# insight-platform/Similari

Hardware: NVIDIA H100
Metric: pair_associations_per_sec (higher is better)
Workload: dtype f32

## Files before the change

### similari_b200/csrc/kernels_feat_tc.cu

```cuda
#include <cuda.h>
#include <cuda_bf16.h>
#include <cuda_runtime.h>
#include <stdint.h>

#include <algorithm>
#include <cstdlib>
#include <cstring>

#include "sb_engine.cuh"
#include "sb_tc.cuh"

namespace sb {

constexpr int TC_STAGES = 4;
constexpr int TC_STAGE_BYTES = TC_A_BYTES + TC_B_BYTES;

struct TcHdr { int scene, m0, ncols_left, m, det_base, col0, epoch, vis_lbase, vis_lcap, pad; };
struct TcSmem {
  unsigned char stage[TC_STAGES][TC_STAGE_BYTES];
  VisColMeta meta[4][TC_BN];
  VisRowMeta rowm[4][TC_BM];
  float colb[4][TC_BN];
  unsigned int colvalid[4][TC_BN / 32];
  TcHdr hdr[4];
  unsigned long long full_bar[TC_STAGES];
  unsigned long long empty_bar[TC_STAGES];
  unsigned long long meta_full[4];
  unsigned long long meta_empty[4];
};
static_assert(sizeof(TcSmem) + 1024 <= 227 * 1024, "screen kernel exceeds the shared memory of an SM");


template <bool COSINE>
__global__ void __launch_bounds__(TC_THREADS, 1)
vis_screen_kernel(const __grid_constant__ CUtensorMap mapA, const __grid_constant__ CUtensorMap mapB, Params p,
                  TrackStore ts, Frame f, const TcTile* tiles, int n_tiles_host, const int* n_tiles_dev,
                  const VisColMeta* colmeta, const VisColGeo* colgeo, const VisRowMeta* rowmeta, const float* colb,
                  const unsigned int* colvalid) {
  const int n_tiles = n_tiles_dev ? *n_tiles_dev : n_tiles_host;
  extern __shared__ unsigned char smem_raw_[];
  TcSmem& S = *reinterpret_cast<TcSmem*>(smem_raw_ + ((1024u - (smem_u32(smem_raw_) & 1023u)) & 1023u));
  const int warp = threadIdx.x >> 5, lane = threadIdx.x & 31;
  const int K = p.max_obs;
  const int KB = (p.d8 + TC_BK - 1) / TC_BK;

  unsigned char* const stage_base = &S.stage[0][0];
  const uint32_t crank = cluster_rank();
  const int cta_first = (int)(blockIdx.x >> 1);
  const int cta_step = (int)(gridDim.x >> 1);
  if (threadIdx.x == 0) {
    for (int s = 0; s < TC_STAGES; ++s) { mbar_init(&S.full_bar[s], 1); mbar_init(&S.empty_bar[s], 4); }
    for (int b = 0; b < 4; ++b) { mbar_init(&S.meta_full[b], 1); mbar_init(&S.meta_empty[b], 8); }
    asm volatile("fence.mbarrier_init.release.cluster;" ::: "memory");
  }
  __syncthreads();
  cluster_sync_all();

  if (warp < 4) {
    asm volatile("setmaxnreg.dec.sync.aligned.u32 40;");
    if (warp == 0 && lane == 0) {
      asm volatile("prefetch.tensormap [%0];" ::"l"((uint64_t)&mapA) : "memory");
      asm volatile("prefetch.tensormap [%0];" ::"l"((uint64_t)&mapB) : "memory");
      int stage = 0;
      uint32_t phase = 0;
      int it = 0;
      TcTile tl_n;
      tl_n.scene = 0; tl_n.m0 = 0; tl_n.c0 = 0; tl_n.pad = 0;
      if (cta_first < n_tiles) tl_n = tiles[cta_first];
      SceneDesc sc_n = f.scenes[tl_n.scene];
      for (int t = cta_first; t < n_tiles; t += cta_step, ++it) {
        const TcTile tl = tl_n;
        const SceneDesc sc = sc_n;
        if (t + cta_step < n_tiles) { tl_n = tiles[t + cta_step]; sc_n = f.scenes[tl_n.scene]; }
        const int m0 = tl.m0 + (int)crank * TC_BM;
        const int rowA = sc.det_base + m0;
        const int rowB = sc.slot * ts.track_cap * K + tl.c0;
        {
          const int g = it & 3;
          mbar_wait(&S.meta_empty[g], ((it >> 2) & 1) ^ 1);
          TcHdr h;
          h.scene = tl.scene; h.m0 = m0; h.ncols_left = sc.nb * K - tl.c0; h.m = sc.m; h.det_base = sc.det_base;
          h.col0 = sc.col_off + tl.c0; h.epoch = (int)sc.epoch; h.vis_lbase = sc.vis_lbase; h.vis_lcap = sc.vis_lcap; h.pad = 0;
          S.hdr[g] = h;
          mbar_expect_tx(&S.meta_full[g], (uint32_t)(sizeof(VisColMeta) * TC_BN + sizeof(VisRowMeta) * TC_BM +
                                                    4 * TC_BN + TC_BN / 8));
          bulk_load(S.meta[g], colmeta + h.col0, (uint32_t)(sizeof(VisColMeta) * TC_BN), &S.meta_full[g]);
          bulk_load(S.rowm[g], rowmeta + rowA, (uint32_t)(sizeof(VisRowMeta) * TC_BM), &S.meta_full[g]);
          bulk_load(S.colb[g], colb + h.col0, 4 * TC_BN, &S.meta_full[g]);
          bulk_load(S.colvalid[g], colvalid + (h.col0 >> 5), TC_BN / 8, &S.meta_full[g]);
        }
        for (int kb = 0; kb < KB; ++kb) {
          mbar_wait(&S.empty_bar[stage], phase ^ 1);
          unsigned char* base = stage_base + stage * TC_STAGE_BYTES;
          mbar_expect_tx(&S.full_bar[stage], TC_STAGE_BYTES);
          tma_load_2d(base, &mapA, kb * TC_BK, rowA, &S.full_bar[stage]);
          tma_load_2d_mc(base + TC_A_BYTES + crank * (TC_B_BYTES / 2), &mapB, kb * TC_BK, rowB + (int)crank * (TC_BN / 2),
                         &S.full_bar[stage], (uint16_t)0x3);
          if (++stage == TC_STAGES) { stage = 0; phase ^= 1; }
        }
      }
    }
  } else {
    asm volatile("setmaxnreg.inc.sync.aligned.u32 232;");
    const int wg = (warp >> 2) - 1;
    const int rr[2] = {wg * TC_WG_ROWS + (warp & 3) * 16 + (lane >> 2), wg * TC_WG_ROWS + (warp & 3) * 16 + (lane >> 2) + 8};
    const int q2 = 2 * (lane & 3);
    const bool geo = p.n_constraints > 0;
    int stage = 0;
    uint32_t phase = 0;
    int it = 0;
    for (int t = cta_first; t < n_tiles; t += cta_step, ++it) {
      float acc[128];
      tc_consume_tile<2, TC_STAGES, TC_STAGE_BYTES>(acc, stage_base, S.full_bar, S.empty_bar, KB, wg, stage, phase);
      const int ms = it & 3;
      mbar_wait(&S.meta_full[ms], (it >> 2) & 1);
      const VisColMeta* gmeta = S.meta[ms];
      const TcHdr h = S.hdr[ms];
      const float* gcolb = S.colb[ms];
      float rowk[2];
      bool row_ok[2];
      int g[2];
#pragma unroll
      for (int hr = 0; hr < 2; ++hr) {
        const VisRowMeta rm = S.rowm[ms][rr[hr]];
        const int m = h.m0 + rr[hr];
        row_ok[hr] = m < h.m && rm.ok;
        g[hr] = h.det_base + m;
        rowk[hr] = rm.rowk;
      }
      unsigned int keep[4] = {0u, 0u, 0u, 0u};
#pragma unroll
      for (int j = 0; j < TC_BN / 8; ++j) {
        const int c0 = 8 * j + q2;
        const float2 cb = *reinterpret_cast<const float2*>(gcolb + c0);
        const unsigned int vw = S.colvalid[ms][c0 >> 5] >> (c0 & 31);
#pragma unroll
        for (int e = 0; e < 4; ++e) {
          const int hr = e >> 1, cl = e & 1;
          const float b = COSINE ? rowk[hr] * (cl ? cb.y : cb.x) : rowk[hr] + (cl ? cb.y : cb.x);
          const bool k = !(acc[4 * j + e] < b) && ((vw >> cl) & 1u) && c0 + cl < h.ncols_left && row_ok[hr];
          if (k) keep[j >> 3] |= 1u << (((4 * j) & 31) + e);
        }
      }
      if (geo) {
        float cx[2], cy[2], cr[2];
#pragma unroll
        for (int hr = 0; hr < 2; ++hr) {
          cx[hr] = 0.0f; cy[hr] = 0.0f; cr[hr] = 0.0f;
          if (row_ok[hr]) { cx[hr] = f.c_box[(size_t)g[hr] * 6]; cy[hr] = f.c_box[(size_t)g[hr] * 6 + 1]; cr[hr] = f.c_radius[g[hr]]; }
        }
#pragma unroll
        for (int w = 0; w < 4; ++w) {
          unsigned int kk = keep[w];
          while (kk) {
            const int b = __ffs(kk) - 1;
            kk &= kk - 1;
            const int i = w * 32 + b, hr = (i >> 1) & 1;
            const int col = 8 * (i >> 2) + q2 + (i & 1);
            const VisColGeo cg = colgeo[h.col0 + col];
            if (!compat_ok(p, (unsigned int)h.epoch, cg.tep, cx[hr], cy[hr], cr[hr], cg.tx, cg.ty, cg.tr)) keep[w] &= ~(1u << b);
          }
        }
      }
      int cnt = 0;
#pragma unroll
      for (int w = 0; w < 4; ++w) cnt += __popc(keep[w]);
      if (__any_sync(0xffffffffu, cnt != 0)) {
        int incl = cnt;
#pragma unroll
        for (int o = 1; o < 32; o <<= 1) {
          int tt = __shfl_up_sync(0xffffffffu, incl, o);
          if (lane >= o) incl += tt;
        }
        const int total = __shfl_sync(0xffffffffu, incl, 31);
        int base = 0;
        if (lane == 31) base = atomicAdd(&f.vis_cnt[h.scene], total);
        base = __shfl_sync(0xffffffffu, base, 31);
        int pos = base + incl - cnt;
#pragma unroll
        for (int hr = 0; hr < 2; ++hr) {
#pragma unroll
          for (int w = 0; w < 4; ++w) {
            unsigned int kk = keep[w] & (hr ? 0xccccccccu : 0x33333333u);
            while (kk) {
              const int b = __ffs(kk) - 1;
              kk &= kk - 1;
              if (pos < h.vis_lcap) {
                const int i = w * 32 + b;
                const VisColMeta cm = gmeta[8 * (i >> 2) + q2 + (i & 1)];
                VisPair vp;
                vp.g = g[hr]; vp.row = cm.row; vp.scene = h.scene; vp.outcol = cm.outcol;
                f.vis_pairs[h.vis_lbase + pos] = vp;
              }
              ++pos;
            }
          }
        }
      }
      __syncwarp();
      if (lane == 0) mbar_arrive(&S.meta_empty[ms]);
    }
  }
  __syncthreads();
  cluster_sync_all();
}

constexpr int SA_BN = 128;
constexpr int SA_KMAX = 8;
constexpr int SA_A_BLOCK = TC_BM * TC_BK * 2;
constexpr int SA_B_STAGE = SA_BN * TC_BK * 2;
constexpr int SA_STAGES = 5;
constexpr int SA_SLABS = 4;
struct SaHdr { int scene, m0, ncols, m, det_base, col0, epoch, vis_lbase, vis_lcap, unit, last, pad; };
struct SaSmem {
  unsigned char a[SA_KMAX][SA_A_BLOCK];
  unsigned char b[SA_STAGES][SA_B_STAGE];
  VisColMeta meta[SA_SLABS][SA_BN];
  float colb[SA_SLABS][SA_BN];
  float colsb[SA_SLABS][SA_BN];
  unsigned int colvalid[SA_SLABS][SA_BN / 32];
  SaHdr hdr[SA_SLABS];
  unsigned long long a_full[SA_KMAX];
  unsigned long long a_empty;
  unsigned long long full_bar[SA_STAGES];
  unsigned long long empty_bar[SA_STAGES];
  unsigned long long meta_full[SA_SLABS];
  unsigned long long meta_empty[SA_SLABS];
};
static_assert(sizeof(SaSmem) + 1024 <= 227 * 1024, "A-stationary screen kernel exceeds the shared memory of an SM");
constexpr int kScreenStationaryMaxD8 = SA_KMAX * TC_BK;

template <bool COSINE, bool FP8>
__global__ void __launch_bounds__(TC_THREADS, 1)
vis_screen_sa_kernel(const __grid_constant__ CUtensorMap mapA, const __grid_constant__ CUtensorMap mapB, Params p,
                     TrackStore ts, Frame f, const TcTile* units, int n_units_host, const int* n_units_dev, int ucols,
                     const VisColMeta* colmeta, const VisColGeo* colgeo, const VisRowMeta* rowmeta, const float* colb,
                     const float* colsb, const unsigned int* colvalid) {
  constexpr bool kScaled = FP8 && !COSINE;
  constexpr int BKF = FP8 ? 2 * TC_BK : TC_BK;
  const int n_units = n_units_dev ? *n_units_dev : n_units_host;
  extern __shared__ unsigned char smem_raw_[];
  SaSmem& S = *reinterpret_cast<SaSmem*>(smem_raw_ + ((1024u - (smem_u32(smem_raw_) & 1023u)) & 1023u));
  const int warp = threadIdx.x >> 5, lane = threadIdx.x & 31;
  const int K = p.max_obs;
  const int KB = (p.d8 + BKF - 1) / BKF;
  const uint32_t crank = cluster_rank();
  if (threadIdx.x == 0) {
    for (int kb = 0; kb < SA_KMAX; ++kb) mbar_init(&S.a_full[kb], 1);
    mbar_init(&S.a_empty, 2);
    for (int s = 0; s < SA_STAGES; ++s) { mbar_init(&S.full_bar[s], 1); mbar_init(&S.empty_bar[s], 2); }
    for (int b = 0; b < SA_SLABS; ++b) { mbar_init(&S.meta_full[b], 1); mbar_init(&S.meta_empty[b], 4); }
    asm volatile("fence.mbarrier_init.release.cluster;" ::: "memory");
  }
  __syncthreads();
  cluster_sync_all();

  if (warp < 4) {
    asm volatile("setmaxnreg.dec.sync.aligned.u32 40;");
    if (warp == 0 && lane == 0) {
      asm volatile("prefetch.tensormap [%0];" ::"l"((uint64_t)&mapA) : "memory");
      asm volatile("prefetch.tensormap [%0];" ::"l"((uint64_t)&mapB) : "memory");
      int seq = 0, gk = 0, unit = 0;
      for (int u = (int)(blockIdx.x >> 1); u < n_units; u += (int)(gridDim.x >> 1), ++unit) {
        const TcTile tl = units[u];
        const SceneDesc sc = f.scenes[tl.scene];
        const int m0 = tl.m0 + (int)crank * TC_BM;
        const int rowA = sc.det_base + m0;
        const int cols = min(ucols, sc.nb * K - tl.c0);
        const int nct = (cols + SA_BN - 1) / SA_BN;
        const int rowB = sc.slot * ts.track_cap * K + tl.c0;
        if (unit > 0) mbar_wait(&S.a_empty, (unit - 1) & 1);
        if (nct == 1) mbar_arrive(&S.a_empty);
        for (int ct = 0; ct < nct; ++ct, ++seq) {
          const int g = seq % SA_SLABS;
          mbar_wait(&S.meta_empty[g], ((seq / SA_SLABS) & 1) ^ 1);
          SaHdr h;
          h.scene = tl.scene; h.m0 = m0; h.ncols = min(SA_BN, cols - ct * SA_BN); h.m = sc.m; h.det_base = sc.det_base;
          h.col0 = sc.col_off + tl.c0 + ct * SA_BN; h.epoch = (int)sc.epoch; h.vis_lbase = sc.vis_lbase;
          h.vis_lcap = sc.vis_lcap; h.unit = unit; h.last = ct + 2 >= nct; h.pad = 0;
          S.hdr[g] = h;
          mbar_expect_tx(&S.meta_full[g], (uint32_t)(sizeof(VisColMeta) * SA_BN + (kScaled ? 8 : 4) * SA_BN + SA_BN / 8));
          bulk_load(S.meta[g], colmeta + h.col0, (uint32_t)(sizeof(VisColMeta) * SA_BN), &S.meta_full[g]);
          bulk_load(S.colb[g], colb + h.col0, 4 * SA_BN, &S.meta_full[g]);
          if (kScaled) bulk_load(S.colsb[g], colsb + h.col0, 4 * SA_BN, &S.meta_full[g]);
          bulk_load(S.colvalid[g], colvalid + (h.col0 >> 5), SA_BN / 8, &S.meta_full[g]);
          for (int kb = 0; kb < KB; ++kb, ++gk) {
            if (ct == 0) {
              mbar_expect_tx(&S.a_full[kb], SA_A_BLOCK);
              tma_load_2d(S.a[kb], &mapA, kb * BKF, rowA, &S.a_full[kb]);
            }
            const int s = gk % SA_STAGES;
            mbar_wait(&S.empty_bar[s], ((gk / SA_STAGES) & 1) ^ 1);
            mbar_expect_tx(&S.full_bar[s], SA_B_STAGE);
            tma_load_2d_mc(S.b[s] + crank * (SA_B_STAGE / 2), &mapB, kb * BKF, rowB + ct * SA_BN + (int)crank * (SA_BN / 2),
                           &S.full_bar[s], (uint16_t)0x3);
          }
        }
      }
      for (int e = 0; e < 2; ++e, ++seq) {
        const int g = seq % SA_SLABS;
        mbar_wait(&S.meta_empty[g], ((seq / SA_SLABS) & 1) ^ 1);
        S.hdr[g].scene = -1 - e;
        mbar_arrive(&S.meta_full[g]);
      }
    }
  } else {
    asm volatile("setmaxnreg.inc.sync.aligned.u32 232;");
    const int wg = (warp >> 2) - 1;
    const int rr[2] = {(warp & 3) * 16 + (lane >> 2), (warp & 3) * 16 + (lane >> 2) + 8};
    const int q2 = 2 * (lane & 3);
    const bool geo = p.n_constraints > 0;
    const bool elected = (threadIdx.x & 127) == 0;
    for (int pos = wg;; pos += 2) {
      const int ms = pos % SA_SLABS;
      mbar_wait(&S.meta_full[ms], (pos / SA_SLABS) & 1);
      const SaHdr h = S.hdr[ms];
      if (pos > 0) wg2_bar_sync(1 + (pos & 1));
      if (h.scene < 0) {
        if (h.scene == -1) wg2_bar_arrive(1 + ((pos + 1) & 1));
        break;
      }
      float rowk[2][2], rowi[2][2];
      bool row_ok[2][2];
#pragma unroll
      for (int hh = 0; hh < 2; ++hh)
#pragma unroll
        for (int hr = 0; hr < 2; ++hr) {
          const int m = h.m0 + 64 * hh + rr[hr];
          const VisRowMeta rm = rowmeta[h.det_base + m];
          rowk[hh][hr] = rm.rowk;
          rowi[hh][hr] = rm.rowi;
          row_ok[hh][hr] = m < h.m && rm.ok;
        }

      float acc[128];
      {
        const int g0 = pos * KB;
        int stage = g0 % SA_STAGES;
        uint32_t phase = (g0 / SA_STAGES) & 1;
        int prev = -1;
        auto release = [&](int s) {
          if (elected)
            for (uint32_t r = 0; r < 2; ++r) mbar_arrive_cluster(cluster_addr(&S.empty_bar[s], r));
        };
        for (int kb = 0; kb < KB; ++kb) {
          mbar_wait(&S.a_full[kb], (uint32_t)h.unit & 1u);
          mbar_wait(&S.full_bar[stage], phase);
          const uint32_t a0 = smem_u32(S.a[kb]);
          const uint32_t b0 = smem_u32(S.b[stage]);
          wgmma_fence();
#pragma unroll
          for (int k = 0; k < 4; ++k) {
            const uint32_t acc_on = (kb | k) != 0 ? 1u : 0u;
            if (FP8) {
              wgmma_e4m3_m64n128(acc, wgmma_desc(a0 + k * 32), wgmma_desc(b0 + k * 32), acc_on);
              wgmma_e4m3_m64n128(acc + 64, wgmma_desc(a0 + 64 * 128 + k * 32), wgmma_desc(b0 + k * 32), acc_on);
            } else {
              wgmma_bf16_m64n128(acc, wgmma_desc(a0 + k * 32), wgmma_desc(b0 + k * 32), acc_on);
              wgmma_bf16_m64n128(acc + 64, wgmma_desc(a0 + 64 * 128 + k * 32), wgmma_desc(b0 + k * 32), acc_on);
            }
          }
          wgmma_commit();
          wgmma_wait<1>();
          if (prev >= 0) release(prev);
          prev = stage;
          if (++stage == SA_STAGES) { stage = 0; phase ^= 1; }
        }
        wg2_bar_arrive(1 + ((pos + 1) & 1));
        wgmma_wait<0>();
        wgmma_fence_acc(acc);
        release(prev);
        if (h.last && elected) mbar_arrive(&S.a_empty);
      }

      const VisColMeta* gmeta = S.meta[ms];
      const float* gcolb = S.colb[ms];
      unsigned int colm[2] = {0u, 0u};
#pragma unroll
      for (int j = 0; j < SA_BN / 8; ++j) {
        const int c0 = 8 * j + q2;
        unsigned int m2 = (S.colvalid[ms][c0 >> 5] >> (c0 & 31)) & 3u;
        m2 &= (c0 < h.ncols ? 1u : 0u) | (c0 + 1 < h.ncols ? 2u : 0u);
        colm[j >> 3] |= (m2 | (m2 << 2)) << ((4 * j) & 31);
      }
      unsigned int keep[4];
#pragma unroll
      for (int hh = 0; hh < 2; ++hh) {
        const unsigned int rowm = (row_ok[hh][0] ? 0x33333333u : 0u) | (row_ok[hh][1] ? 0xccccccccu : 0u);
        keep[2 * hh] = 0u;
        keep[2 * hh + 1] = 0u;
#pragma unroll
        for (int j = 0; j < SA_BN / 8; ++j) {
          const float2 cb = *reinterpret_cast<const float2*>(gcolb + 8 * j + q2);
          float2 cs = make_float2(1.0f, 1.0f);
          if (kScaled) cs = *reinterpret_cast<const float2*>(&S.colsb[ms][8 * j + q2]);
#pragma unroll
          for (int e = 0; e < 4; ++e) {
            const float rk = rowk[hh][e >> 1], c = (e & 1) ? cb.y : cb.x;
            if (kScaled) {
              const float b = __fmaf_rn((e & 1) ? cs.y : cs.x, rk, c);
              if (!(acc[64 * hh + 4 * j + e] * rowi[hh][e >> 1] < b)) keep[2 * hh + (j >> 3)] |= 1u << ((4 * j + e) & 31);
            } else {
              const float b = COSINE ? rk * c : rk + c;
              if (!(acc[64 * hh + 4 * j + e] < b)) keep[2 * hh + (j >> 3)] |= 1u << ((4 * j + e) & 31);
            }
          }
        }
        keep[2 * hh] &= colm[0] & rowm;
        keep[2 * hh + 1] &= colm[1] & rowm;
      }
      if (geo) {
        float cx[2][2], cy[2][2], cr[2][2];
#pragma unroll
        for (int hh = 0; hh < 2; ++hh)
#pragma unroll
          for (int hr = 0; hr < 2; ++hr) {
            cx[hh][hr] = 0.0f; cy[hh][hr] = 0.0f; cr[hh][hr] = 0.0f;
            if (row_ok[hh][hr]) {
              const size_t g = (size_t)h.det_base + h.m0 + 64 * hh + rr[hr];
              cx[hh][hr] = f.c_box[g * 6]; cy[hh][hr] = f.c_box[g * 6 + 1]; cr[hh][hr] = f.c_radius[g];
            }
          }
#pragma unroll
        for (int w = 0; w < 4; ++w) {
          unsigned int kk = keep[w];
          while (kk) {
            const int b = __ffs(kk) - 1;
            kk &= kk - 1;
            const int i = (w & 1) * 32 + b, hh = w >> 1;
            const bool r8 = (i >> 1) & 1;
            const int col = 8 * (i >> 2) + q2 + (i & 1);
            const VisColGeo cg = colgeo[h.col0 + col];
            if (!compat_ok(p, (unsigned int)h.epoch, cg.tep, r8 ? cx[hh][1] : cx[hh][0], r8 ? cy[hh][1] : cy[hh][0],
                           r8 ? cr[hh][1] : cr[hh][0], cg.tx, cg.ty, cg.tr))
              keep[w] &= ~(1u << b);
          }
        }
      }
      int cnt = 0;
#pragma unroll
      for (int w = 0; w < 4; ++w) cnt += __popc(keep[w]);
      if (__any_sync(0xffffffffu, cnt != 0)) {
        int incl = cnt;
#pragma unroll
        for (int o = 1; o < 32; o <<= 1) {
          int tt = __shfl_up_sync(0xffffffffu, incl, o);
          if (lane >= o) incl += tt;
        }
        const int total = __shfl_sync(0xffffffffu, incl, 31);
        int base = 0;
        if (lane == 31) base = atomicAdd(&f.vis_cnt[h.scene], total);
        base = __shfl_sync(0xffffffffu, base, 31);
        int at = base + incl - cnt;
#pragma unroll
        for (int hh = 0; hh < 2; ++hh) {
#pragma unroll
          for (int hr = 0; hr < 2; ++hr) {
            const int g = h.det_base + h.m0 + 64 * hh + rr[hr];
#pragma unroll
            for (int w = 0; w < 2; ++w) {
              unsigned int kk = keep[2 * hh + w] & (hr ? 0xccccccccu : 0x33333333u);
              while (kk) {
                const int b = __ffs(kk) - 1;
                kk &= kk - 1;
                if (at < h.vis_lcap) {
                  const int i = w * 32 + b;
                  const VisColMeta cm = gmeta[8 * (i >> 2) + q2 + (i & 1)];
                  VisPair vp;
                  vp.g = g; vp.row = cm.row; vp.scene = h.scene; vp.outcol = cm.outcol;
                  f.vis_pairs[h.vis_lbase + at] = vp;
                }
                ++at;
              }
            }
          }
        }
      }
      __syncwarp();
      if (lane == 0) mbar_arrive(&S.meta_empty[ms]);
    }
  }
  __syncthreads();
  cluster_sync_all();
}


constexpr int RF_WARPS = 4;
constexpr int RF_SEG = 64;
constexpr int RF_PITCH = RF_SEG + 1;
constexpr int RF_CLAIM = 16;

template <bool TAIL>
__device__ __forceinline__ void refine_load_a(const float* __restrict__ a, int blk, int D, float* av) {
  if (!TAIL) {
    const float4 a0 = *reinterpret_cast<const float4*>(a + blk * 8);
    const float4 a1 = *reinterpret_cast<const float4*>(a + blk * 8 + 4);
    av[0] = a0.x; av[1] = a0.y; av[2] = a0.z; av[3] = a0.w; av[4] = a1.x; av[5] = a1.y; av[6] = a1.z; av[7] = a1.w;
  } else {
#pragma unroll
    for (int l = 0; l < 8; ++l) av[l] = blk * 8 + l < D ? a[blk * 8 + l] : 0.0f;
  }
}
template <bool TAIL, class T>
__device__ __forceinline__ void refine_load_a(const T* __restrict__ a, int blk, int D, float* av) {
  if (!TAIL) {
    feat_widen8(*reinterpret_cast<const uint4*>(a + blk * 8), a, av);
  } else {
#pragma unroll
    for (int l = 0; l < 8; ++l) av[l] = blk * 8 + l < D ? feat_elem(a, blk * 8 + l) : 0.0f;
  }
}
template <bool COSINE>
__device__ __forceinline__ float refine_block_sum(const float* av, const float* __restrict__ b, int blk) {
  const float4 b0 = *reinterpret_cast<const float4*>(b + blk * 8);
  const float4 b1 = *reinterpret_cast<const float4*>(b + blk * 8 + 4);
  const float bb[8] = {b0.x, b0.y, b0.z, b0.w, b1.x, b1.y, b1.z, b1.w};
  float t[8];
#pragma unroll
  for (int l = 0; l < 8; ++l) {
    if (COSINE) t[l] = av[l] * bb[l];
    else { const float df = av[l] - bb[l]; t[l] = df * df; }
  }
  return reduce_add8(t);
}

template <bool COSINE, bool TAIL, class T>
__global__ void __launch_bounds__(RF_WARPS * 32, 8) vis_refine_kernel(Params p, TrackStore ts, Frame f, int* nan_flag,
                                                                      int n_scenes) {
  __shared__ float s_bs[RF_WARPS][RF_CLAIM][RF_PITCH];
  __shared__ int s_cnt[2];
  for (int scene = blockIdx.y; scene < n_scenes; scene += gridDim.y) {
    if (f.vis_mode[scene] != 0) {
      if (f.screen_cnt && blockIdx.x == 0 && threadIdx.x == 0) atomicAdd(f.screen_cnt + 2, 1);
      continue;
    }
    const SceneDesc sc = f.scenes[scene];
    const int lane = threadIdx.x & 31, w = threadIdx.x >> 5;
    if (f.screen_cnt) {
      if (threadIdx.x < 2) s_cnt[threadIdx.x] = 0;
      __syncthreads();
    }
    int n_ref = 0, n_cut = 0;
    const int n_pairs = min(f.vis_cnt[scene], sc.vis_lcap);
    const int nblk = p.d8 / 8;
    const int D = p.feature_dim;
    float (*bs)[RF_PITCH] = s_bs[w];
    float vmax = nanf("");
    for (;;) {
      int i0 = 0;
      if (lane == 0) i0 = atomicAdd(f.refine_next + scene, RF_CLAIM);
      i0 = __shfl_sync(0xffffffffu, i0, 0);
      if (i0 >= n_pairs) break;
      const int npair = min(RF_CLAIM, n_pairs - i0);
      VisPair mine;
      mine.g = 0; mine.row = 0; mine.scene = 0; mine.outcol = 0;
      if (lane < npair) mine = f.vis_pairs[sc.vis_lbase + i0 + lane];
      float acc = 0.0f;
      for (int seg0 = 0; seg0 < nblk; seg0 += RF_SEG) {
        const int segn = min(RF_SEG, nblk - seg0);
        int g_prev = -1;
        float av[RF_SEG / 32][8];
#pragma unroll 4
        for (int pp = 0; pp < npair; ++pp) {
          const int g = __shfl_sync(0xffffffffu, mine.g, pp);
          const int row = __shfl_sync(0xffffffffu, mine.row, pp);
          const float* b = ts.feat + (size_t)row * p.d8;
          if (g != g_prev) {
            const T* a = static_cast<const T*>(f.in_feat) + (size_t)g * D;
#pragma unroll
            for (int h = 0; h < RF_SEG / 32; ++h)
              if (h * 32 + lane < segn) refine_load_a<TAIL>(a, seg0 + h * 32 + lane, D, av[h]);
            g_prev = g;
          }
#pragma unroll
          for (int h = 0; h < RF_SEG / 32; ++h) {
            const int j = h * 32 + lane;
            if (j < segn) bs[pp][j] = refine_block_sum<COSINE>(av[h], b, seg0 + j);
          }
        }
        __syncwarp();
        if (lane < npair)
          for (int j = 0; j < segn; ++j) acc = acc + bs[lane][j];
        __syncwarp();
      }
      if (lane < npair) {
        float v = nanf("");
        if (COSINE) {
          const float d = acc / sqrtf(f.c_norm2[mine.g] * ts.fnorm2[mine.row]);
          if (d >= p.visual_threshold) v = 1.0f - d;
        } else {
          const float d = sqrtf(acc);
          if (d <= p.visual_threshold) v = d;
        }
        f.vis_val[sc.vis_lbase + i0 + lane] = v;
        n_ref += 1;
        n_cut += is_nan(v) ? 1 : 0;
        if (!is_nan(v) && !(v <= vmax)) vmax = v;
        if (nan_flag && is_nan(v)) nan_flag[scene] = 1;
      }
    }
    unsigned int u = 0u;
    if (!is_nan(vmax)) {
      u = __float_as_uint(vmax);
      u = (u & 0x80000000u) ? ~u : (u | 0x80000000u);
    }
#pragma unroll
    for (int o = 16; o > 0; o >>= 1) u = max(u, __shfl_xor_sync(0xffffffffu, u, o));
    if (lane == 0 && u != 0u) atomicMax(f.scene_max + scene, u);
    if (f.screen_cnt) {
      n_ref = __reduce_add_sync(0xffffffffu, n_ref);
      n_cut = __reduce_add_sync(0xffffffffu, n_cut);
      if (lane == 0 && n_ref) { atomicAdd(&s_cnt[0], n_ref); atomicAdd(&s_cnt[1], n_cut); }
      __syncthreads();
      if (threadIdx.x == 0 && s_cnt[0]) { atomicAdd(f.screen_cnt, s_cnt[0]); if (s_cnt[1]) atomicAdd(f.screen_cnt + 1, s_cnt[1]); }
      __syncthreads();
    }
  }
}

__global__ void vis_fill_none_kernel(Params p, Frame f, int n_scenes) {
  for (int scene = blockIdx.y; scene < n_scenes; scene += gridDim.y) {
    if (f.scene_mode[scene] != 0) continue;
    const SceneDesc sc = f.scenes[scene];
    const long long cnt = (long long)sc.m * sc.n * p.max_obs;
    float* out = f.vis + sc.vis_off;
    const float qnan = nanf("");
    for (long long i = (long long)blockIdx.x * blockDim.x + threadIdx.x; i < cnt; i += (long long)gridDim.x * blockDim.x) out[i] = qnan;
  }
}
__global__ void vis_scatter_kernel(Params p, Frame f, int n_scenes) {
  for (int scene = blockIdx.y; scene < n_scenes; scene += gridDim.y) {
    if (f.scene_mode[scene] != 0) continue;
    const SceneDesc sc = f.scenes[scene];
    const int n_pairs = min(f.vis_cnt[scene], sc.vis_lcap);
    float* out = f.vis + sc.vis_off;
    for (int i = blockIdx.x * blockDim.x + threadIdx.x; i < n_pairs; i += gridDim.x * blockDim.x) {
      const VisPair vp = f.vis_pairs[sc.vis_lbase + i];
      out[(size_t)(vp.g - sc.det_base) * (sc.n * p.max_obs) + vp.outcol] = f.vis_val[sc.vis_lbase + i];
    }
  }
}
void launch_vis_densify(const Params& p, const Frame& f, int n_scenes, cudaStream_t st) {
  if (n_scenes == 0) return;
  dim3 grid(64, scene_grid(n_scenes));
  vis_fill_none_kernel<<<grid, 256, 0, st>>>(p, f, n_scenes);
  vis_scatter_kernel<<<grid, 256, 0, st>>>(p, f, n_scenes);
  note_launch(2);
}

__global__ void to_bf16_kernel(const float* src, int src_pitch, int d, int d8, long long rows, __nv_bfloat16* dst) {
  long long i = (long long)blockIdx.x * blockDim.x + threadIdx.x;
  if (i >= rows * d8) return;
  long long r = i / d8;
  int c = (int)(i - r * d8);
  float x = c < d ? src[r * src_pitch + c] : 0.0f;
  dst[i] = __float2bfloat16_rn(x);
}

void launch_to_bf16(const float* src, int src_pitch, int d, int d8, long long rows, void* dst, cudaStream_t st) {
  if (rows == 0) return;
  long long n = rows * d8;
  to_bf16_kernel<<<(unsigned)((n + 255) / 256), 256, 0, st>>>(src, src_pitch, d, d8, rows, (__nv_bfloat16*)dst);
  note_launch();
}

__global__ void to_fp8_kernel(const float* src, int src_pitch, int d, int d8, long long rows, unsigned char* dst, float* scale) {
  const long long r = ((long long)blockIdx.x * blockDim.x + threadIdx.x) >> 5;
  if (r >= rows) return;
  const float s = fp8_row_from(src + r * src_pitch, d, d8, dst + r * fp8_pitch(d8));
  if ((threadIdx.x & 31) == 0) scale[r] = s;
}

void launch_to_fp8(const float* src, int src_pitch, int d, int d8, long long rows, unsigned char* dst, float* scale,
                   cudaStream_t st) {
  if (rows == 0) return;
  to_fp8_kernel<<<(unsigned)((rows * 32 + 255) / 256), 256, 0, st>>>(src, src_pitch, d, d8, rows, dst, scale);
  note_launch();
}

typedef CUresult (*EncodeTiledFn)(CUtensorMap*, CUtensorMapDataType, cuuint32_t, void*, const cuuint64_t*, const cuuint64_t*,
                                  const cuuint32_t*, const cuuint32_t*, CUtensorMapInterleave, CUtensorMapSwizzle,
                                  CUtensorMapL2promotion, CUtensorMapFloatOOBfill);

static EncodeTiledFn get_encode() {
  static EncodeTiledFn fn = nullptr;
  if (!fn) {
    void* p = nullptr;
    cudaDriverEntryPointQueryResult qr;
    if (cudaGetDriverEntryPoint("cuTensorMapEncodeTiled", &p, cudaEnableDefault, &qr) == cudaSuccess && p) fn = (EncodeTiledFn)p;
  }
  return fn;
}

int make_map(CUtensorMap* m, const void* base, long long rows, int d8, int box_rows, bool fp8) {
  EncodeTiledFn enc = get_encode();
  if (!enc) return -1;
  cuuint64_t dims[2] = {(cuuint64_t)d8, (cuuint64_t)rows};
  cuuint64_t strides[1] = {fp8 ? (cuuint64_t)fp8_pitch(d8) : (cuuint64_t)d8 * 2};
  cuuint32_t box[2] = {(cuuint32_t)(fp8 ? 2 * TC_BK : TC_BK), (cuuint32_t)box_rows};
  cuuint32_t estr[2] = {1, 1};
  CUresult r = enc(m, fp8 ? CU_TENSOR_MAP_DATA_TYPE_UINT8 : CU_TENSOR_MAP_DATA_TYPE_BFLOAT16, 2, (void*)base, dims, strides, box, estr, CU_TENSOR_MAP_INTERLEAVE_NONE,
                   CU_TENSOR_MAP_SWIZZLE_128B, CU_TENSOR_MAP_L2_PROMOTION_L2_256B, CU_TENSOR_MAP_FLOAT_OOB_FILL_NONE);
  return r == CUDA_SUCCESS ? 0 : -2;
}

static bool screen_fp8(const Params& p, const TcArgs& tc) { return tc.fp8 && !tc.dense && p.d8 <= kFp8MaxD8; }

__global__ void vis_meta_kernel(Params p, TrackStore ts, Frame f, int n_scenes, int max_rows, VisColMeta* colmeta,
                                VisColGeo* colgeo, float* colb, float* colsb, unsigned int* colvalid, bool fp8) {
  for (int s = blockIdx.y; s < n_scenes; s += gridDim.y) {
    const SceneDesc sc = f.scenes[s];
    const int K = p.max_obs;
    const int prow = blockIdx.x * blockDim.x + threadIdx.x;
    const bool in = prow < sc.nb * K && prow < max_rows;
    VisColMeta cm;
    cm.colb = 0.0f; cm.colc = 0.0f; cm.outcol = -1; cm.row = -1;
    float csb = 1.0f;
    if (in) {
      const int b = prow / K, ph = prow - b * K;
      const size_t sbase = (size_t)sc.slot * ts.track_cap;
      const int n = ts.blk_owner ? ts.blk_owner[sbase + b] : b;
      const size_t ti = sbase + (n >= 0 ? n : 0);
      const size_t frow = (sbase + b) * K + ph;
      unsigned int tep = 0u;
      if (n >= 0) {
        const int on = ts.obs_n[ti];
        int k_of = -1, live_mask = 0;
        for (int k = 0; k < K; ++k) {
          if (k < on && ts.obs_hasf[ti * K + k]) {
            int pp = ts.obs_phys[ti * K + k];
            live_mask |= 1 << pp;
            if (pp == ph) k_of = k;
          }
        }
        tep = ts.epoch[ti];
        if (k_of >= 0) {
          const unsigned int delta = sc.epoch > tep ? sc.epoch - tep : tep - sc.epoch;
          cm.outcol = n * K + k_of;
          const bool valid = (ts.feat_cnt[ti] >= p.min_track_length) && ((unsigned int)p.max_idle_epochs >= delta);
          const float nb = ts.fnorm2[frow];
          const float E = fp8 ? p.vis_rel_err8 : p.vis_rel_err;
          cm.colb = p.visual_kind == 1 ? sqrtf(nb) : 0.5f * nb * (1.0f - 1e-5f - E);
          if (fp8) {
            if (fp8_norm_ok(nb)) { csb = ts.fscale[frow]; cm.colb *= csb; }
            else cm.colb = nanf("");
          }
          cm.row = valid ? (int)frow : -1;
        } else {
          int dead_rank = 0;
          for (int pp = 0; pp < ph; ++pp) dead_rank += ((live_mask >> pp) & 1) ? 0 : 1;
          int seen = 0;
          for (int k = 0; k < K; ++k) {
            bool lv = k < on && ts.obs_hasf[ti * K + k];
            if (!lv) { if (seen == dead_rank) { cm.outcol = n * K + k; break; } ++seen; }
          }
        }
      }
      colmeta[sc.col_off + prow] = cm;
      colb[sc.col_off + prow] = cm.colb;
      if (fp8 && p.visual_kind != 1) colsb[sc.col_off + prow] = csb;
      if (p.n_constraints > 0) {
        VisColGeo cg;
        cg.tx = 0.0f; cg.ty = 0.0f; cg.tr = 0.0f; cg.tep = tep;
        if (n >= 0) { const float* tb = ts.pred + ti * 6; cg.tx = tb[0]; cg.ty = tb[1]; cg.tr = ts.radius[ti]; }
        colgeo[sc.col_off + prow] = cg;
      }
    }
    const unsigned int vb = __ballot_sync(0xffffffffu, cm.row >= 0);
    if ((threadIdx.x & 31) == 0 && vb != 0) colvalid[(sc.col_off + prow) >> 5] = vb;
    else if ((threadIdx.x & 31) == 0 && in) colvalid[(sc.col_off + prow) >> 5] = 0u;
  }
}

__global__ void vis_rowmeta_kernel(Params p, Frame f, VisRowMeta* rowmeta, bool fp8) {
  int g = blockIdx.x * blockDim.x + threadIdx.x;
  if (g >= f.total) return;
  g += f.det0;
  const float na = f.c_norm2[g];
  VisRowMeta rm;
  rm.ok = (f.c_flags[g] & 2) ? 1 : 0;
  rm.rowi = 1.0f;
  rm.pad = 0;
  const float thr = p.visual_threshold;
  const float E = fp8 ? p.vis_rel_err8 : p.vis_rel_err;
  if (p.visual_kind == 1) rm.rowk = (thr - 1e-5f - E) * sqrtf(na);
  else rm.rowk = 0.5f * (na * (1.0f - 1e-5f - E) - thr * thr * (1.0f + 1e-5f));
  if (fp8) {
    const float s = f.c_scale[g];
    if (!fp8_norm_ok(na)) rm.rowk = nanf("");
    else if (p.visual_kind == 1) rm.rowk *= s;
    else rm.rowi = 1.0f / s;
  }
  rowmeta[g] = rm;
}

int launch_vis_refine(const Params& p, const TrackStore& ts, const Frame& f, int n_scenes, int* nan_flag, cudaStream_t st) {
  if (n_scenes == 0) return 0;
  dim3 grid(16, scene_grid(n_scenes));
  const bool tail = p.feature_dim != p.d8 || (reinterpret_cast<uintptr_t>(f.in_feat) & 15) != 0;
  feat_dispatch(f.feat_type, [&](auto t) {
    using T = decltype(t);
    if (p.visual_kind == 1) {
      if (tail) vis_refine_kernel<true, true, T><<<grid, RF_WARPS * 32, 0, st>>>(p, ts, f, nan_flag, n_scenes);
      else vis_refine_kernel<true, false, T><<<grid, RF_WARPS * 32, 0, st>>>(p, ts, f, nan_flag, n_scenes);
    } else {
      if (tail) vis_refine_kernel<false, true, T><<<grid, RF_WARPS * 32, 0, st>>>(p, ts, f, nan_flag, n_scenes);
      else vis_refine_kernel<false, false, T><<<grid, RF_WARPS * 32, 0, st>>>(p, ts, f, nan_flag, n_scenes);
    }
  });
  note_launch();
  return 0;
}

void launch_vis_colmeta(const Params& p, const TrackStore& ts, const Frame& f, int n_scenes, int max_n, const TcArgs& tc,
                        cudaStream_t st) {
  const int max_rows = tc.max_rows > 0 ? tc.max_rows : max_n * p.max_obs;
  if (tc.n_tiles == 0 || max_rows <= 0) return;
  dim3 grid((max_rows + 255) / 256, scene_grid(n_scenes));
  vis_meta_kernel<<<grid, 256, 0, st>>>(p, ts, f, n_scenes, max_rows, tc.colmeta, tc.colgeo, tc.colb, tc.colsb, tc.colvalid,
                                        screen_fp8(p, tc));
  note_launch();
}

int vis_screen_ucols(int d8, int num_sms, int n_scenes, const int* m, const int* nb, int K) {
  if (d8 > kScreenStationaryMaxD8) return TC_BN;
  long long pairs = 0, pair_tiles = 0;
  int max_ct = 1;
  for (int s = 0; s < n_scenes; ++s) {
    const int ct = (nb[s] * K + SA_BN - 1) / SA_BN, rp = (m[s] + 2 * TC_BM - 1) / (2 * TC_BM);
    pairs += rp;
    pair_tiles += (long long)rp * ct;
    max_ct = std::max(max_ct, ct);
  }
  const long long units = 2ll * std::max(1, num_sms / 2);
  if (pairs >= units) return max_ct * SA_BN;
  const long long per = (pair_tiles + units - 1) / units;
  return (int)std::max<long long>(2, std::min<long long>(per, max_ct)) * SA_BN;
}

int launch_vis_cost_tc(const Params& p, const TrackStore& ts, const Frame& f, int n_scenes, int max_n, const TcArgs& tc,
                       int phase, cudaStream_t st) {
  if (tc.n_tiles == 0) return 0;
  if (phase == 1) {
    int rc = launch_vis_refine(p, ts, f, n_scenes, tc.dense ? tc.dense_bad : nullptr, st);
    if (tc.ev_refine1) cudaEventRecord(tc.ev_refine1, st);
    return rc;
  }
  const bool stationary = p.d8 <= kScreenStationaryMaxD8;
  const bool fp8 = screen_fp8(p, tc);
  if (fp8 && (!f.c_fp8 || !f.c_scale || !ts.feat_fp8 || !ts.fscale || (p.visual_kind != 1 && !tc.colsb))) return -3;
  CUtensorMap mA, mB;
  if (make_map(&mA, fp8 ? (const void*)f.c_fp8 : f.c_bf16, tc.a_rows, p.d8, TC_BM, fp8) ||
      make_map(&mB, fp8 ? (const void*)ts.feat_fp8 : ts.feat_bf16, tc.b_rows, p.d8, stationary ? SA_BN / 2 : TC_BN / 2, fp8))
    return -1;
  const size_t smem = (stationary ? sizeof(SaSmem) : sizeof(TcSmem)) + 1024;
  const bool cosine = p.visual_kind == 1;
  cudaError_t e = cudaSuccess;
  const void* fn;
  if (!stationary) fn = cosine ? (const void*)vis_screen_kernel<true> : (const void*)vis_screen_kernel<false>;
  else if (fp8) fn = cosine ? (const void*)vis_screen_sa_kernel<true, true> : (const void*)vis_screen_sa_kernel<false, true>;
  else fn = cosine ? (const void*)vis_screen_sa_kernel<true, false> : (const void*)vis_screen_sa_kernel<false, false>;
  e = cudaFuncSetAttribute(fn, cudaFuncAttributeMaxDynamicSharedMemorySize, (int)smem);
  if (e != cudaSuccess) return (int)e;
  if (!tc.colmeta_done) launch_vis_colmeta(p, ts, f, n_scenes, max_n, tc, st);
  vis_rowmeta_kernel<<<(f.total + 255) / 256, 256, 0, st>>>(p, f, tc.rowmeta, fp8);
  note_launch();
  if (tc.ev_screen0) cudaEventRecord(tc.ev_screen0, st);
  {
    const int ncta = 2 * std::min(tc.n_tiles, tc.num_sms / 2);
    cudaLaunchConfig_t cfg;
    memset(&cfg, 0, sizeof(cfg));
    cfg.gridDim = dim3(ncta);
    cfg.blockDim = dim3(TC_THREADS);
    cfg.dynamicSmemBytes = smem;
    cfg.stream = st;
    cudaLaunchAttribute attr[1];
    attr[0].id = cudaLaunchAttributeClusterDimension;
    attr[0].val.clusterDim.x = 2; attr[0].val.clusterDim.y = 1; attr[0].val.clusterDim.z = 1;
    cfg.attrs = attr;
    cfg.numAttrs = 1;
    const TcTile* d_tiles = tc.d_tiles;
    int n_tiles = tc.n_tiles;
    const int* d_n_tiles = tc.d_n_tiles;
    const VisColMeta* cmeta = tc.colmeta;
    const VisColGeo* cgeo = tc.colgeo;
    const VisRowMeta* rmeta = tc.rowmeta;
    const float* cb = tc.colb;
    const float* csb = tc.colsb;
    const unsigned int* cv = tc.colvalid;
    int ucols = tc.cstep;
    void* args[] = {(void*)&mA, (void*)&mB, (void*)&p, (void*)&ts, (void*)&f, (void*)&d_tiles, (void*)&n_tiles,
                    (void*)&d_n_tiles, (void*)&cmeta, (void*)&cgeo, (void*)&rmeta, (void*)&cb, (void*)&cv};
    void* args_sa[] = {(void*)&mA, (void*)&mB, (void*)&p, (void*)&ts, (void*)&f, (void*)&d_tiles, (void*)&n_tiles,
                       (void*)&d_n_tiles, (void*)&ucols, (void*)&cmeta, (void*)&cgeo, (void*)&rmeta, (void*)&cb, (void*)&csb,
                       (void*)&cv};
    e = cudaLaunchKernelExC(&cfg, fn, stationary ? args_sa : args);
    if (e != cudaSuccess) return (int)e;
    note_launch();
  }
  if (tc.ev_screen1) cudaEventRecord(tc.ev_screen1, st);
  return 0;
}

}
```

Before: 61.40 billion.

## Defer sparse pair writes past next GEMM and cache row metadata per unit

In the FP8 A-stationary screen kernel, row metadata is now reloaded only when the work unit changes, not for every column slab. When every lane has at most two surviving pairs, those pairs are stashed in registers and written out after the next tile's wgmma issue, so the global stores overlap tensor-core work. Optional phase-timing instrumentation is also added behind a compile flag. The cost is extra live registers in the consumer warps and a more complex, easier-to-break output path.

```diff
diff --git a/similari_b200/csrc/kernels_feat_tc.cu b/similari_b200/csrc/kernels_feat_tc.cu
--- a/similari_b200/csrc/kernels_feat_tc.cu
+++ b/similari_b200/csrc/kernels_feat_tc.cu
@@ -230,6 +230,19 @@
 static_assert(sizeof(SaSmem) + 1024 <= 227 * 1024, "A-stationary screen kernel exceeds the shared memory of an SM");
 constexpr int kScreenStationaryMaxD8 = SA_KMAX * TC_BK;
 
+#ifdef SB_SCREEN_PHASES
+constexpr int kSaPhaseCtas = 1024, kSaPhaseSlots = 32;
+__device__ unsigned long long g_sa_phase[kSaPhaseCtas][kSaPhaseSlots];
+__device__ __forceinline__ unsigned long long sa_gtime() {
+  unsigned long long t;
+  asm volatile("mov.u64 %0, %%globaltimer;" : "=l"(t));
+  return t;
+}
+#define SA_PH(...) __VA_ARGS__
+#else
+#define SA_PH(...)
+#endif
+
 template <bool COSINE, bool FP8>
 __global__ void __launch_bounds__(TC_THREADS, 1)
 vis_screen_sa_kernel(const __grid_constant__ CUtensorMap mapA, const __grid_constant__ CUtensorMap mapB, Params p,
@@ -254,12 +267,15 @@
   }
   __syncthreads();
   cluster_sync_all();
+  SA_PH(unsigned long long* const ph_row = g_sa_phase[blockIdx.x];
+        if (threadIdx.x == 0) { ph_row[20] = sa_gtime(); ph_row[24] = clock64(); })
 
   if (warp < 4) {
     asm volatile("setmaxnreg.dec.sync.aligned.u32 40;");
     if (warp == 0 && lane == 0) {
       asm volatile("prefetch.tensormap [%0];" ::"l"((uint64_t)&mapA) : "memory");
       asm volatile("prefetch.tensormap [%0];" ::"l"((uint64_t)&mapB) : "memory");
+      SA_PH(unsigned long long pw[3] = {0, 0, 0}; long long pt;)
       int seq = 0, gk = 0, unit = 0;
       for (int u = (int)(blockIdx.x >> 1); u < n_units; u += (int)(gridDim.x >> 1), ++unit) {
         const TcTile tl = units[u];
@@ -269,11 +285,15 @@
         const int cols = min(ucols, sc.nb * K - tl.c0);
         const int nct = (cols + SA_BN - 1) / SA_BN;
         const int rowB = sc.slot * ts.track_cap * K + tl.c0;
+        SA_PH(pt = clock64();)
         if (unit > 0) mbar_wait(&S.a_empty, (unit - 1) & 1);
+        SA_PH(pw[1] += clock64() - pt;)
         if (nct == 1) mbar_arrive(&S.a_empty);
         for (int ct = 0; ct < nct; ++ct, ++seq) {
           const int g = seq % SA_SLABS;
+          SA_PH(pt = clock64();)
           mbar_wait(&S.meta_empty[g], ((seq / SA_SLABS) & 1) ^ 1);
+          SA_PH(pw[2] += clock64() - pt;)
           SaHdr h;
           h.scene = tl.scene; h.m0 = m0; h.ncols = min(SA_BN, cols - ct * SA_BN); h.m = sc.m; h.det_base = sc.det_base;
           h.col0 = sc.col_off + tl.c0 + ct * SA_BN; h.epoch = (int)sc.epoch; h.vis_lbase = sc.vis_lbase;
@@ -290,7 +310,9 @@
               tma_load_2d(S.a[kb], &mapA, kb * BKF, rowA, &S.a_full[kb]);
             }
             const int s = gk % SA_STAGES;
+            SA_PH(pt = clock64();)
             mbar_wait(&S.empty_bar[s], ((gk / SA_STAGES) & 1) ^ 1);
+            SA_PH(pw[0] += clock64() - pt;)
             mbar_expect_tx(&S.full_bar[s], SA_B_STAGE);
             tma_load_2d_mc(S.b[s] + crank * (SA_B_STAGE / 2), &mapB, kb * BKF, rowB + ct * SA_BN + (int)crank * (SA_BN / 2),
                            &S.full_bar[s], (uint16_t)0x3);
@@ -303,6 +325,7 @@
         S.hdr[g].scene = -1 - e;
         mbar_arrive(&S.meta_full[g]);
       }
+      SA_PH(ph_row[0] += pw[0]; ph_row[1] += pw[1]; ph_row[2] += pw[2]; ph_row[3] += unit;)
     }
   } else {
     asm volatile("setmaxnreg.inc.sync.aligned.u32 232;");
@@ -311,27 +334,50 @@
     const int q2 = 2 * (lane & 3);
     const bool geo = p.n_constraints > 0;
     const bool elected = (threadIdx.x & 127) == 0;
+    SA_PH(unsigned long long cw[7] = {0, 0, 0, 0, 0, 0, 0}, cw_test = 0, n_t = 0, g_last = 0; long long ct0 = clock64(), ct1;)
+    float rowk[2][2], rowi[2][2];
+    bool row_ok[2][2];
+    int row_unit = -1;
+    constexpr bool kStash = FP8;
+    bool st_any = false;
+    int st_n = 0, st_ex = 0, st_base = 0, st_scene = 0, st_lbase = 0, st_lcap = 0;
+    int st_g0 = 0, st_row0 = 0, st_oc0 = 0, st_g1 = 0, st_row1 = 0, st_oc1 = 0;
+    auto flush = [&]() {
+      if (!st_any) return;
+      int b31;
+      asm volatile("mov.b32 %0, %1;" : "=r"(b31) : "r"(st_base));
+      const int at = __shfl_sync(0xffffffffu, b31, 31) + st_ex;
+      VisPair vp;
+      vp.scene = st_scene;
+      if (st_n > 0 && at < st_lcap) { vp.g = st_g0; vp.row = st_row0; vp.outcol = st_oc0; f.vis_pairs[st_lbase + at] = vp; }
+      if (st_n > 1 && at + 1 < st_lcap) { vp.g = st_g1; vp.row = st_row1; vp.outcol = st_oc1; f.vis_pairs[st_lbase + at + 1] = vp; }
+      st_any = false;
+    };
     for (int pos = wg;; pos += 2) {
       const int ms = pos % SA_SLABS;
       mbar_wait(&S.meta_full[ms], (pos / SA_SLABS) & 1);
+      SA_PH(ct1 = clock64(); cw[0] += ct1 - ct0; ct0 = ct1;)
       const SaHdr h = S.hdr[ms];
       if (pos > 0) wg2_bar_sync(1 + (pos & 1));
+      SA_PH(ct1 = clock64(); cw[1] += ct1 - ct0; ct0 = ct1;)
       if (h.scene < 0) {
         if (h.scene == -1) wg2_bar_arrive(1 + ((pos + 1) & 1));
+        if (kStash) flush();
         break;
       }
-      float rowk[2][2], rowi[2][2];
-      bool row_ok[2][2];
-#pragma unroll
-      for (int hh = 0; hh < 2; ++hh)
-#pragma unroll
-        for (int hr = 0; hr < 2; ++hr) {
-          const int m = h.m0 + 64 * hh + rr[hr];
-          const VisRowMeta rm = rowmeta[h.det_base + m];
-          rowk[hh][hr] = rm.rowk;
-          rowi[hh][hr] = rm.rowi;
-          row_ok[hh][hr] = m < h.m && rm.ok;
-        }
+      if (!FP8 || h.unit != row_unit) {
+        row_unit = h.unit;
+#pragma unroll
+        for (int hh = 0; hh < 2; ++hh)
+#pragma unroll
+          for (int hr = 0; hr < 2; ++hr) {
+            const int m = h.m0 + 64 * hh + rr[hr];
+            const VisRowMeta rm = rowmeta[h.det_base + m];
+            rowk[hh][hr] = rm.rowk;
+            rowi[hh][hr] = rm.rowi;
+            row_ok[hh][hr] = m < h.m && rm.ok;
+          }
+      }
 
       float acc[128];
       {
@@ -344,8 +390,11 @@
             for (uint32_t r = 0; r < 2; ++r) mbar_arrive_cluster(cluster_addr(&S.empty_bar[s], r));
         };
         for (int kb = 0; kb < KB; ++kb) {
+          SA_PH(long long wt = clock64();)
           mbar_wait(&S.a_full[kb], (uint32_t)h.unit & 1u);
+          SA_PH(const long long wt1 = clock64(); cw[2] += wt1 - wt; wt = wt1;)
           mbar_wait(&S.full_bar[stage], phase);
+          SA_PH(cw[3] += clock64() - wt;)
           const uint32_t a0 = smem_u32(S.a[kb]);
           const uint32_t b0 = smem_u32(S.b[stage]);
           wgmma_fence();
@@ -367,11 +416,14 @@
           if (++stage == SA_STAGES) { stage = 0; phase ^= 1; }
         }
         wg2_bar_arrive(1 + ((pos + 1) & 1));
+        SA_PH(ct1 = clock64(); cw[4] += ct1 - ct0; ct0 = ct1;)
         wgmma_wait<0>();
         wgmma_fence_acc(acc);
+        SA_PH(ct1 = clock64(); cw[5] += ct1 - ct0; ct0 = ct1; g_last = sa_gtime(); ++n_t;)
         release(prev);
         if (h.last && elected) mbar_arrive(&S.a_empty);
       }
+      if (kStash) flush();
 
       const VisColMeta* gmeta = S.meta[ms];
       const float* gcolb = S.colb[ms];
@@ -437,6 +489,7 @@
           }
         }
       }
+      SA_PH(cw_test += clock64() - ct0;)
       int cnt = 0;
 #pragma unroll
       for (int w = 0; w < 4; ++w) cnt += __popc(keep[w]);
@@ -450,6 +503,25 @@
         const int total = __shfl_sync(0xffffffffu, incl, 31);
         int base = 0;
         if (lane == 31) base = atomicAdd(&f.vis_cnt[h.scene], total);
+        if (kStash && __all_sync(0xffffffffu, cnt <= 2)) {
+          st_any = true; st_n = cnt; st_ex = incl - cnt; st_base = base;
+          st_scene = h.scene; st_lbase = h.vis_lbase; st_lcap = h.vis_lcap;
+          int j = 0;
+#pragma unroll
+          for (int w = 0; w < 4; ++w) {
+            unsigned int kk = keep[w];
+            while (kk) {
+              const int b = __ffs(kk) - 1;
+              kk &= kk - 1;
+              const int i = (w & 1) * 32 + b;
+              const int g = h.det_base + h.m0 + 64 * (w >> 1) + (((i >> 1) & 1) ? rr[1] : rr[0]);
+              const VisColMeta cm = gmeta[8 * (i >> 2) + q2 + (i & 1)];
+              if (j == 0) { st_g0 = g; st_row0 = cm.row; st_oc0 = cm.outcol; }
+              else { st_g1 = g; st_row1 = cm.row; st_oc1 = cm.outcol; }
+              ++j;
+            }
+          }
+        } else {
         base = __shfl_sync(0xffffffffu, base, 31);
         int at = base + incl - cnt;
 #pragma unroll
@@ -475,14 +547,34 @@
             }
           }
         }
+        }
       }
       __syncwarp();
       if (lane == 0) mbar_arrive(&S.meta_empty[ms]);
-    }
+      SA_PH(ct1 = clock64(); cw[6] += ct1 - ct0; ct0 = ct1;)
+    }
+    SA_PH(if (elected) {
+      for (int i = 0; i < 7; ++i) ph_row[4 + 7 * wg + i] += cw[i];
+      ph_row[18 + wg] += n_t;
+      ph_row[21 + wg] = g_last;
+      ph_row[26 + wg] += cw_test;
+    })
   }
   __syncthreads();
   cluster_sync_all();
-}
+  SA_PH(if (threadIdx.x == 0) { ph_row[23] = sa_gtime(); ph_row[25] = clock64(); })
+}
+
+#ifdef SB_SCREEN_PHASES
+}
+extern "C" int sb200_screen_phases(unsigned long long* out, int n_ctas) {
+  const size_t bytes = sizeof(unsigned long long) * sb::kSaPhaseSlots * (size_t)std::min(n_ctas, sb::kSaPhaseCtas);
+  if (cudaMemcpyFromSymbol(out, sb::g_sa_phase, bytes) != cudaSuccess) return -1;
+  static unsigned long long zeros[sb::kSaPhaseCtas][sb::kSaPhaseSlots];
+  return cudaMemcpyToSymbol(sb::g_sa_phase, zeros, sizeof(zeros)) == cudaSuccess ? 0 : -1;
+}
+namespace sb {
+#endif
 
 
 constexpr int RF_WARPS = 4;
```

After: 62.06 billion, median of 6. 1.01x the previous value.
